# mFinn27/Template-Matching-and-Regression-MapReduce

Hardware: AMD Instinct MI355X
Metric: images/sec (whole node) match+regress+NMS; % HBM/MFMA roofline at 1/2/4/8 GPU (higher is better)
Workload: dtype fp32; 1 GPU; config B: 64x SAM feats 256x64x64 (->128x128), 3 exemplars, templates 3x3-15x15, fp32, cls 0.1, IoU 0.5; config=B, images_per_gpu=64, exemplars=3, parallelism=dp1, decoder=split, decoder_precision=fp32

## Files before the change

### template-matching-and-regression-mapreduce_amd/csrc/conv_split.hip

```cpp
#include <algorithm>
#include <type_traits>

#include "tmr_common.h"

namespace {

typedef _Float16 h8 __attribute__((ext_vector_type(8)));
typedef __bf16 b8 __attribute__((ext_vector_type(8)));
typedef float f32x4 __attribute__((ext_vector_type(4)));
typedef __bf16 b4 __attribute__((ext_vector_type(4)));
typedef __attribute__((address_space(3))) void *lds_ptr_t;


constexpr int BM = 128;
constexpr int TH = 16;
constexpr int TW = 32;
constexpr int LDS_KB = 160;
constexpr int PXG = 8, NG = 4;
constexpr int NWAVES = 8;
constexpr int NTHREADS = NWAVES * 64;
constexpr int WNS = (NWAVES == 8 || TH == 8) ? 2 : 1;
static_assert(TH == 4 * NWAVES / WNS, "a wave owns 4 output rows");
constexpr int NIN = 8 / WNS;
constexpr int ACCW = NIN * 8 * 64 * 4;
// ... 537 lines not shown
#pragma unroll
            for (int q = 0; q < 4; ++q)
                head_fma(head_act((f2){acc[in][2 * q][r], acc[in][2 * q + 1][r]}, inv2, bn2, a.leaky), hw2, hs2[q]);
            __builtin_amdgcn_sched_barrier(0);
        }
    float X[40];
#pragma unroll
    for (int q = 0; q < 4; ++q)
#pragma unroll
        for (int k = 0; k < NHEAD; ++k) {
            X[2 * (5 * q + k)] = hs2[q][k].x;
            X[2 * (5 * q + k) + 1] = hs2[q][k].y;
        }
    float Y[20], Z[10];
#pragma unroll
    for (int m = 0; m < 20; ++m) {
        const auto s = __builtin_amdgcn_permlane16_swap(__float_as_uint(X[2 * m]), __float_as_uint(X[2 * m + 1]),
                                                         false, false);
        Y[m] = __uint_as_float(s[0]) + __uint_as_float(s[1]);
    }
#pragma unroll
    for (int p = 0; p < 10; ++p) {
        const auto s = __builtin_amdgcn_permlane32_swap(__float_as_uint(Y[2 * p]), __float_as_uint(Y[2 * p + 1]),
                                                         false, false);
        Z[p] = __uint_as_float(s[0]) + __uint_as_float(s[1]);
    }
    __syncthreads();
    if (WNS == 2 && wn == 1) {
#pragma unroll
        for (int p = 0; p < 10; ++p) red[((wpix * 10 + p) * 4 + kg) * 16 + l16] = Z[p];
    }
    __syncthreads();
    if (wn == 0) {
#pragma unroll
        for (int p = 0; p < 10; ++p) {
            const int j = 4 * p + kg, m = j >> 1, q = m / NHEAD, k = m - q * NHEAD;
            const int jp = 2 * q + (j & 1);
            const int y = ty0 + wpix * 4 + (jp >> 1), x = tx0 + (jp & 1) * 16 + l16;
            const float v = Z[p] + (WNS == 2 ? red[((wpix * 10 + p) * 4 + kg) * 16 + l16] : 0.0f);
            if (y < a.H && x < a.W) a.partials[(((size_t)nt * NHEAD + k) * a.U + u) * HW + (size_t)y * a.W + x] = v;
        }
    }
}

template <int KS, int PREC, int EPI>
int launch_split(SArgs a, hipStream_t s) {
    constexpr size_t lds = Geo<KS, PREC>::LDS;
    static_assert(lds <= 160 * 1024, "LDS");
    static_assert((4 * 8 * NHEAD * 16 + BM * (NHEAD + 1)) * 4 <= lds, "epilogue scratch");
    auto kern = split_conv_kernel<KS, PREC, EPI>;
    if (tmr_set_max_lds((const void *)kern, lds) !=
        hipSuccess)
        return TMR_E_HIP;
    const int64_t blocks = (int64_t)a.NTW * a.MT * a.U;
    if (blocks <= 0) return TMR_OK;
    TMR_REQUIRE(blocks < (1ll << 31));
    hipLaunchKernelGGL(kern, dim3((unsigned)blocks), dim3(NTHREADS), lds, s, a);
    TMR_CHECK_LAUNCH();
    return TMR_OK;
}

template <int KS, int EPI>
int dispatch_prec(int prec, const SArgs &a, hipStream_t s) {
    switch (prec) {
        case TMR_PREC_F16X3: return launch_split<KS, TMR_PREC_F16X3, EPI>(a, s);
        case TMR_PREC_BF16: return launch_split<KS, TMR_PREC_BF16, EPI>(a, s);
        case TMR_PREC_F16: return launch_split<KS, TMR_PREC_F16, EPI>(a, s);
        default: return TMR_E_INVALID;
    }
}

template <int EPI>
int dispatch_ks(int ks, int prec, const SArgs &a, hipStream_t s) {
    switch (ks) {
        case 1: return dispatch_prec<1, EPI>(prec, a, s);
        case 3: return dispatch_prec<3, EPI>(prec, a, s);
        case 5: return dispatch_prec<5, EPI>(prec, a, s);
        case 7: return dispatch_prec<7, EPI>(prec, a, s);
        default: return TMR_E_INVALID;
    }
}

constexpr int PT = TMR_POINTS_TILE;
constexpr int PCG = PT / 16;
static_assert(PT == 64 && 4 * PT <= NTHREADS, "points tile: one gather lane per point");

struct PArgs {
    SArgs s;
    const float *head_bias;
    const float *box;
    const int32_t *tiles;
    float *b;
};

template <int KS, int PREC>
__global__ __launch_bounds__(NTHREADS) void split_points_kernel(PArgs pa) {
    typedef Prec<PREC> PR;
    typedef typename PR::V V;
    constexpr int T = KS * KS, HALVES = PR::HALVES, WREC = PR::WREC;
    constexpr int NF = BM / 16;
    constexpr int NS = HALVES == 2 ? 3 * T : T;
    const SArgs &a = pa.s;
    constexpr int BB = T * P * PT * 16;
    extern __shared__ __attribute__((aligned(16))) char plds[];
    char *Bs = plds;
    float(*red)[4][PT] = reinterpret_cast<float(*)[4][PT]>(plds + 2 * BB);

    const int tid = threadIdx.x;
    const int lane = tid & 63;
    const int wave = __builtin_amdgcn_readfirstlane(tid >> 6);
    const int l16 = lane & 15, kg = lane >> 4;
    const int HW = a.H * a.W;
    const int32_t *tl = pa.tiles + 3 * (size_t)blockIdx.x;
    const int u = min(max(tl[0], 0), a.U - 1);
    const int first = min(max(tl[1], 0), HW - 1), cnt = min(max(tl[2], 0), PT);
    const int img = a.unit_image ? a.unit_image[u] : u;
    const int NC = a.NC0 + a.NC1;
    const bool active = wave < a.NTW;
    const int nt = a.NT0 + (active ? wave : 0);
    const int *pixi = reinterpret_cast<const int *>(pa.box) + 4 * (size_t)u * HW;
    auto pixel = [&](int p) { return min(max(pixi[4 * (size_t)min(first + (p < cnt ? p : 0), HW - 1)], 0), HW - 1); };

    {
        int py[PCG], px[PCG];
#pragma unroll
        for (int j = 0; j < PCG; ++j) {
            const int pix = pixel(j * 16 + l16);
            py[j] = pix / a.W;
            px[j] = pix - py[j] * a.W;
        }
        const uint32_t cstride = (uint32_t)a.Hp * a.Wp * XREC;
        const int h0 = a.NC0 * HALVES, h1 = a.NC1 * HALVES;
        const __amdgpu_buffer_rsrc_t xr0 = __builtin_amdgcn_make_buffer_rsrc(
            (void *)(h0 ? a.x0 + (size_t)img * h0 * cstride : a.x1), (short)0, h0 * cstride, 0x00020000);
        const __amdgpu_buffer_rsrc_t xr1 = __builtin_amdgcn_make_buffer_rsrc(
            (void *)(h1 ? a.x1 + (size_t)u * h1 * cstride : a.x0), (short)0, h1 * cstride, 0x00020000);
        const uint32_t tapstride = (uint32_t)NC * a.Npad * WREC;
        const __amdgpu_buffer_rsrc_t wr = __builtin_amdgcn_make_buffer_rsrc(
            (void *)a.wp, (short)0, T * tapstride, 0x00020000);
        const uint32_t aoff = (uint32_t)kg * a.Npad * 16 + ((uint32_t)nt * BM + l16) * 16;
        uint32_t goff;
        {
            const int pix = pixel(lane), y = pix / a.W;
            goff = (uint32_t)(y * a.Wp + (pix - y * a.W)) * 16;
        }
        const uint32_t qstride = (uint32_t)a.Hp * a.Wp * 16;
        auto gather = [&](int hc) {
            const bool s0 = hc < h0;
            const uint32_t hs_ = (uint32_t)(s0 ? hc : hc - h0) * cstride;
#pragma unroll
            for (int m = 0; m < (T * P + NWAVES - 1) / NWAVES; ++m) {
                const int i = wave + NWAVES * m;
                if (i < T * P) {
                    const int tap = i / P, q = i % P, ky = tap / KS, kx = tap % KS;
                    buffer_lds16(s0 ? xr0 : xr1, (lds_ptr_t)(Bs + (hc & 1) * BB + i * (PT * 16)), goff,
                                 hs_ + q * qstride + (uint32_t)(ky * a.Wp + kx) * 16);
                }
            }
        };
        const int bfo = kg * (PT * 16) + l16 * 16;
        auto bfrag = [&](int hc, int tap, int j) -> V {
            return *reinterpret_cast<const V *>(Bs + (hc & 1) * BB + tap * (P * PT * 16) + bfo + j * 256);
        };
        gather(0);

        const float sxw = split_sxw<PREC>(a, u);
        f32x4 acc[NF][PCG];
        if (a.acc_init) {
            const int islab = (a.flags & TMR_SPLIT_INIT_BCAST) ? 0 : img;
            const bool i16 = a.flags & TMR_SPLIT_INIT_BF16;
#pragma unroll
            for (int j = 0; j < PCG; ++j) {
                const int mt = (py[j] / TH) * a.TXN + px[j] / TW;
                const int wpix = (py[j] % TH) >> 2, jp = ((py[j] & 3) << 1) | ((px[j] % TW) >> 4);
                const size_t g4 = (((((size_t)islab * a.NT + nt) * a.MT + mt) * NWAVES + wpix * WNS) * ACCW) / 4 +
                                  jp * 64 + kg * 16 + (px[j] & 15);
                if (i16) {
                    const b4 *ai = reinterpret_cast<const b4 *>(a.acc_init) + g4;
#pragma unroll
                    for (int f = 0; f < NF; ++f)
                        acc[f][j] = __builtin_convertvector(ai[(f / NIN) * (ACCW / 4) + (f % NIN) * 8 * 64], f32x4) * sxw;
                } else {
                    const f32x4 *ai = reinterpret_cast<const f32x4 *>(a.acc_init) + g4;
#pragma unroll
                    for (int f = 0; f < NF; ++f)
                        acc[f][j] = ai[(f / NIN) * (ACCW / 4) + (f % NIN) * 8 * 64] * sxw;
                }
            }
        } else {
#pragma unroll
            for (int f = 0; f < NF; ++f)
#pragma unroll
                for (int j = 0; j < PCG; ++j) acc[f][j] = (f32x4){0.0f, 0.0f, 0.0f, 0.0f};
        }

        auto st_part = [](int s) { return HALVES == 2 && s >= 2 * T ? 1 : 0; };
        auto st_tap = [](int s) { return HALVES == 2 ? (s >= 2 * T ? s - 2 * T : s / 2) : s; };
        auto st_term = [](int s) { return HALVES == 2 && s < 2 * T ? s & 1 : 0; };
        auto st_newb = [](int s) { return !(HALVES == 2 && s < 2 * T && (s & 1)); };
        auto st_first = [](int s) { return s == 0 || (HALVES == 2 && s == 2 * T); };
        auto st_last = [](int s) { return s == NS - 1 || (HALVES == 2 && s == 2 * T - 1); };
        V an[NF], bn[PCG];
        auto load_stage = [&](int c, int s) {
            const int tap = st_tap(s);
            const uint32_t as = (uint32_t)tap * tapstride + (uint32_t)c * a.Npad * WREC +
                                (uint32_t)st_term(s) * 4 * a.Npad * 16;
#pragma unroll
            for (int f = 0; f < NF; ++f) an[f] = buffer_load16<V>(wr, aoff + f * 256, as);
            if (st_newb(s) && !st_first(s)) {
#pragma unroll
                for (int j = 0; j < PCG; ++j) bn[j] = bfrag(c * HALVES + st_part(s), tap, j);
            }
        };
        load_stage(0, 0);
        asm volatile("s_waitcnt vmcnt(0)" ::: "memory");
        __syncthreads();
        V bc[PCG];
        const int NHC = NC * HALVES;
        for (int c = 0; c < NC; ++c) {
#pragma unroll
            for (int s = 0; s < NS; ++s) {
                const int hc = c * HALVES + st_part(s);
                V ac[NF];
#pragma unroll
                for (int f = 0; f < NF; ++f) ac[f] = an[f];
                if (st_first(s)) {
                    if (hc + 1 < NHC) gather(hc + 1);
#pragma unroll
                    for (int j = 0; j < PCG; ++j) bc[j] = bfrag(hc, st_tap(s), j);
                } else if (st_newb(s)) {
#pragma unroll
                    for (int j = 0; j < PCG; ++j) bc[j] = bn[j];
                }
                if (s + 1 < NS)
                    load_stage(c, s + 1);
                else
                    load_stage(c + 1 < NC ? c + 1 : c, 0);
                __builtin_amdgcn_sched_barrier(0);
#pragma unroll
                for (int j = 0; j < PCG; ++j)
#pragma unroll
                    for (int f = 0; f < NF; ++f) acc[f][j] = mma(ac[f], bc[j], acc[f][j]);
                __builtin_amdgcn_sched_barrier(0);
                if (st_last(s)) {
                    asm volatile("s_waitcnt vmcnt(0)" ::: "memory");
                    __syncthreads();
                }
            }
        }

        const float inv = 1.0f / sxw;
        const f2 inv2 = {inv, inv};
        f2 hs[WNS][PCG / 2][NHEAD];
#pragma unroll
        for (int w = 0; w < WNS; ++w)
#pragma unroll
            for (int q = 0; q < PCG / 2; ++q)
#pragma unroll
                for (int k = 0; k < NHEAD; ++k) hs[w][q][k] = (f2){0.0f, 0.0f};
#pragma unroll
        for (int f = 0; f < NF; ++f)
#pragma unroll
            for (int r = 0; r < 4; ++r) {
                const int n = nt * BM + f * 16 + 4 * kg + r;
                const float bv = n < a.N ? a.bias[n] : 0.0f;
                const f2 bn2 = {bv, bv};
                f2 hw2[NHEAD];
#pragma unroll
                for (int k = 0; k < NHEAD; ++k) {
                    const float h = a.headw[(size_t)n * NHEAD + k];
                    hw2[k] = (f2){h, h};
                }
#pragma unroll
                for (int q = 0; q < PCG / 2; ++q)
                    head_fma(head_act((f2){acc[f][2 * q][r], acc[f][2 * q + 1][r]}, inv2, bn2, a.leaky), hw2,
                             hs[f / NIN][q]);
            }
#pragma unroll
        for (int q = 0; q < PCG / 2; ++q)
#pragma unroll
            for (int k = 0; k < 4; ++k)
#pragma unroll
                for (int e = 0; e < 2; ++e) {
                    float z[WNS];
#pragma unroll
                    for (int w = 0; w < WNS; ++w) {
                        const float x = hs[w][q][k][e];
                        const float y = x + __shfl_xor(x, 16);
                        z[w] = y + __shfl_xor(y, 32);
                    }
                    if (kg == 0 && active) red[wave][k][(2 * q + e) * 16 + l16] = WNS == 2 ? z[0] + z[1] : z[0];
                }
    }
    __syncthreads();
    if (tid < 4 * PT) {
        const int k = tid / PT, p = tid % PT;
        if (p < cnt) {
            const int pix = pixel(p);
            float s = 0.0f;
            for (int t = 0; t < a.NTW; ++t) s += red[t][k][p];
            pa.b[((size_t)u * 4 + k) * HW + pix] = s + pa.head_bias[k];
        }
    }
}

template <int PREC>
int launch_points(const PArgs &pa, int ntiles, hipStream_t s) {
    constexpr size_t lds = 2 * 9 * P * PT * 16 + NWAVES * 4 * PT * sizeof(float);
    auto kern = split_points_kernel<3, PREC>;
    if (tmr_set_max_lds((const void *)kern, lds) != hipSuccess) return TMR_E_HIP;
    hipLaunchKernelGGL(kern, dim3((unsigned)ntiles), dim3(NTHREADS), lds, s, pa);
    TMR_CHECK_LAUNCH();
    return TMR_OK;
}

inline int prec_halves(int prec) { return prec == TMR_PREC_F16X3 ? 2 : 1; }
inline int prec_wrec(int prec) { return prec == TMR_PREC_F16X3 ? 128 : 64; }
inline bool prec_ok(int prec) {
    return prec == TMR_PREC_F16X3 || prec == TMR_PREC_BF16 || prec == TMR_PREC_F16;
}
inline bool ks_ok(int ks) { return ks == 1 || ks == 3 || ks == 5 || ks == 7; }
inline bool tile_window(int flags, int NT, int &first, int &count) {
    first = (flags >> TMR_SPLIT_TILE_FIRST_SHIFT) & 0xff;
    count = (flags >> TMR_SPLIT_TILE_COUNT_SHIFT) & 0x7f;
    if (count == 0) {
        if (first != 0) return false;
        count = NT;
    }
    return first + count <= NT;
}
inline int pad_h(int H, int ks) { return (int)tmr_cdiv(H, TH) * TH + ks - 1; }
inline int pad_w(int W, int ks) { return (int)tmr_cdiv(W, TW) * TW + ks - 1; }

__device__ __forceinline__ void absmax_commit(float m, unsigned *out) {
    __shared__ float red[4];
    for (int o = 32; o > 0; o >>= 1) m = fmaxf(m, __shfl_xor(m, o));
    if ((threadIdx.x & 63) == 0) red[threadIdx.x >> 6] = m;
    __syncthreads();
    if (threadIdx.x == 0) atomicMax(out, __float_as_uint(fmaxf(fmaxf(red[0], red[1]), fmaxf(red[2], red[3]))));
}

__global__ __launch_bounds__(256) void absmax_rows_kernel(const float *__restrict__ x, int64_t n, int vec,
                                                          unsigned *__restrict__ out) {
    const float *xr = x + (size_t)blockIdx.y * n;
    float m = 0.0f;
    const int64_t step = (int64_t)gridDim.x * blockDim.x;
    if (vec) {
        const float4 *x4 = reinterpret_cast<const float4 *>(xr);
        for (int64_t i = (int64_t)blockIdx.x * blockDim.x + threadIdx.x; i < n / 4; i += step) {
            const float4 v = x4[i];
            m = fmaxf(m, fmaxf(fmaxf(fabsf(v.x), fabsf(v.y)), fmaxf(fabsf(v.z), fabsf(v.w))));
        }
    } else {
        for (int64_t i = (int64_t)blockIdx.x * blockDim.x + threadIdx.x; i < n; i += step)
            m = fmaxf(m, fabsf(xr[i]));
    }
    absmax_commit(m, out + blockIdx.y);
}

constexpr int PA_PIX = 64, PA_GRP = 8;
__global__ __launch_bounds__(PA_PIX * PA_GRP) void pixel_absmax_kernel(const float *__restrict__ x, int S, int C,
                                                                       int64_t HW, float *__restrict__ out) {
    __shared__ float part[PA_GRP][PA_PIX];
    const int lane = threadIdx.x & (PA_PIX - 1), grp = threadIdx.x / PA_PIX;
    const int64_t i = (int64_t)blockIdx.x * PA_PIX + lane;
    float m = 0.0f;
    if (i < (int64_t)S * HW) {
        const int64_t s = i / HW, p = i - s * HW;
        const float *xp = x + (size_t)s * C * HW + p;
#pragma unroll 8
        for (int c = grp; c < C; c += PA_GRP) m = fmaxf(m, fabsf(xp[(size_t)c * HW]));
    }
    part[grp][lane] = m;
    __syncthreads();
    if (grp == 0 && i < (int64_t)S * HW) {
#pragma unroll
        for (int g = 1; g < PA_GRP; ++g) m = fmaxf(m, part[g][lane]);
        out[i] = m;
    }
}

__global__ __launch_bounds__(256) void scale_merge_kernel(const float *__restrict__ img_max,
                                                          const float *__restrict__ unit_max,
                                                          const int32_t *__restrict__ unit_image, int U,
                                                          float *__restrict__ out_img,
                                                          float *__restrict__ out_unit) {
    __shared__ float red[4];
    const int b = blockIdx.x;
    float m = 0.0f;
    for (int u = threadIdx.x; u < U; u += blockDim.x)
        if (unit_image[u] == b) m = fmaxf(m, unit_max[u]);
    for (int o = 32; o > 0; o >>= 1) m = fmaxf(m, __shfl_xor(m, o));
    if ((threadIdx.x & 63) == 0) red[threadIdx.x >> 6] = m;
    __syncthreads();
// ... 371 lines not shown
}

extern "C" int tmr_split_wpack(const float *w, int N, int C0, int C1, int ks, int prec,
                               const float *wmax, void *out, void *stream) {
    TMR_REQUIRE(w && out && N > 0 && C0 >= 0 && C1 >= 0 && C0 + C1 > 0 && ks_ok(ks) && prec_ok(prec));
    TMR_REQUIRE(prec == TMR_PREC_BF16 || wmax);
    const int NC0 = (int)tmr_cdiv(C0, CCH), NC = NC0 + (int)tmr_cdiv(C1, CCH);
    const int Npad = (int)tmr_cdiv(N, BM) * BM;
    const int64_t total = (int64_t)ks * ks * NC * Npad;
    const dim3 grid((unsigned)tmr_cdiv(total, 256)), blk(256);
    hipStream_t s = tmr_stream(stream);
    switch (prec) {
        case TMR_PREC_F16X3:
            hipLaunchKernelGGL(wpack_kernel<TMR_PREC_F16X3>, grid, blk, 0, s, w, N, C0, C1, ks, NC0,
                               NC, Npad, wmax, static_cast<h8 *>(out));
            break;
        case TMR_PREC_BF16:
            hipLaunchKernelGGL(wpack_kernel<TMR_PREC_BF16>, grid, blk, 0, s, w, N, C0, C1, ks, NC0,
                               NC, Npad, nullptr, static_cast<b8 *>(out));
            break;
        default:
            hipLaunchKernelGGL(wpack_kernel<TMR_PREC_F16>, grid, blk, 0, s, w, N, C0, C1, ks, NC0,
                               NC, Npad, wmax, static_cast<h8 *>(out));
            break;
    }
    TMR_CHECK_LAUNCH();
    return TMR_OK;
}

extern "C" int tmr_split_conv(const void *xp0, int C0, const int32_t *unit_image, const void *xp1, int C1, int U,
                              int H, int W, int ks, int prec, const void *wpack, const float *wmax, const float *xmax,
                              const float *bias, int N, int leaky, const float *headw, const float *acc_init,
                              float *out, int flags, void *stream) {
    TMR_REQUIRE(out);
    if (!headw)
        return split_common(xp0, C0, unit_image, xp1, C1, U, H, W, ks, prec, wpack, wmax, xmax, bias, N, leaky,
                            acc_init, out, nullptr, nullptr, 0, flags, stream);
    TMR_REQUIRE(!(flags & TMR_SPLIT_TILED_OUT));
    return split_common(xp0, C0, unit_image, xp1, C1, U, H, W, ks, prec, wpack, wmax, xmax, bias, N, leaky, acc_init,
                        nullptr, headw, out, 1, flags, stream);
}

extern "C" int tmr_split_conv_points(const void *xp0, int C0, const int32_t *unit_image, const void *xp1, int C1,
                                     int U, int H, int W, int ks, int prec, const void *wpack, const float *wmax,
                                     const float *xmax, const float *bias, int N, int leaky, const float *headw,
                                     const float *head_bias, const float *acc_init, const float *box,
                                     const int32_t *tiles, int ntiles, float *b, int flags, void *stream) {
    TMR_REQUIRE(prec_ok(prec) && ks_ok(ks));
    TMR_REQUIRE(wpack && bias && headw && head_bias && box && b && U > 0 && H > 0 && W > 0 && N > 0);
    TMR_REQUIRE(C0 >= 0 && C1 >= 0 && C0 + C1 > 0 && (C0 == 0 || xp0) && (C1 == 0 || xp1));
    TMR_REQUIRE(prec == TMR_PREC_BF16 || (wmax && xmax));
    TMR_REQUIRE(ntiles >= 0 && (ntiles == 0 || tiles));
    TMR_REQUIRE(!(flags & (TMR_SPLIT_TILED_OUT | TMR_SPLIT_OUT_BF16 | TMR_SPLIT_XMAX_PER_PIXEL)));
    TMR_REQUIRE(!acc_init || (flags & TMR_SPLIT_TILED_INIT));
    TMR_REQUIRE(!(flags & TMR_SPLIT_INIT_BF16) || ((flags & TMR_SPLIT_TILED_INIT) && prec != TMR_PREC_F16X3));
    TMR_REQUIRE((int64_t)H * W < (1ll << 29));
    PArgs pa = {};
    SArgs &a = pa.s;
    a.x0 = static_cast<const char *>(xp0);
    a.x1 = static_cast<const char *>(xp1);
    a.unit_image = unit_image;
    a.wp = static_cast<const char *>(wpack);
    a.wmax = prec == TMR_PREC_BF16 ? nullptr : wmax;
    a.xmax = prec == TMR_PREC_BF16 ? nullptr : xmax;
    a.bias = bias;
    a.headw = headw;
    a.acc_init = acc_init;
    a.NC0 = (int)tmr_cdiv(C0, CCH);
    a.NC1 = (int)tmr_cdiv(C1, CCH);
    a.U = U;
    a.H = H;
    a.W = W;
    a.N = N;
    a.NT = (int)tmr_cdiv(N, BM);
    a.Npad = a.NT * BM;
    a.TXN = (int)tmr_cdiv(W, TW);
    a.MT = a.TXN * (int)tmr_cdiv(H, TH);
    a.Hp = pad_h(H, ks);
    a.Wp = pad_w(W, ks);
    a.leaky = leaky;
    a.flags = flags & 0xff;
    a.EI = 1;
    TMR_REQUIRE(tile_window(flags, a.NT, a.NT0, a.NTW));
    if (ks != 3 || a.NTW > NWAVES) return TMR_E_UNSUPPORTED;
    pa.head_bias = head_bias;
    pa.box = box;
    pa.tiles = tiles;
    pa.b = b;
    if (ntiles == 0) return TMR_OK;
    hipStream_t s = tmr_stream(stream);
    switch (prec) {
        case TMR_PREC_F16X3: return launch_points<TMR_PREC_F16X3>(pa, ntiles, s);
        case TMR_PREC_BF16: return launch_points<TMR_PREC_BF16>(pa, ntiles, s);
        default: return launch_points<TMR_PREC_F16>(pa, ntiles, s);
    }
}
```

### template-matching-and-regression-mapreduce_amd/engine.py

```python
from __future__ import annotations

import contextlib
import weakref
from dataclasses import dataclass
from typing import Dict, Optional, Sequence, Tuple

import numpy as np
import torch

from . import exp_table, graphs, host
from ._lib import (PEAKS_DECODE_ONLY, PEAKS_FIND_ONLY, PEAKS_PROB_SCRATCH, POINTS_TILE, PREC_CODES, SPLIT_OUT_BF16,
                   SPLIT_TILED_OUT, SPLIT_XMAX_PER_PIXEL, UNIT_DTYPE, XCORR_ALGOS, TMRError, call, ptr, require_gpu,
                   size, stream, xcorr)
from .decoder_plan import SCALES_FTM, SCALES_MERGED, HeadsLaunch, decoder_plan
from .graphs import _clone_outputs, _GraphBook, _h2d, _units_to_device
from .operands import absmax
from .operands import (absmax_rows, conv2d_split, fold_proj, pack_split_up, pack_split_w, pack_split_x, pixel_absmax,
                       prec_code, scale_merge)
from .xcorr_cost import mfma_fits, xcorr_choice

NHEAD = 5
NMS_SMALL = 256


# ... 266 lines not shown
        self.last_xcorr_flops = float(np.sum(2.0 * C * (H - ht + 1) * (W - wt + 1) * ht * wt))
        self.last_xcorr_bytes = 2.0 * 4 * C * H * W * U
        nimg = len(set(int(i) for i in unit_image))
        self.last_xcorr_dram_bytes = float(C * H * W) * (4.0 * nimg + (2.0 if out16 else 4.0) * U)
        self._memo_absmax(out, "ftm", lambda: slots)
        return out, relu

    def decode(self, fp: torch.Tensor, f_tm: torch.Tensor, unit_image: Sequence[int],
               feats: Optional[torch.Tensor] = None, box_later: bool = False):
        cfg = self.cfg
        ui = _h2d(np.asarray(unit_image, np.int32), f_tm.device, tag="unit_image")
        if cfg.decoder_num_layer != 1:
            return self._decode_stack(fp, f_tm, ui)
        U, C1, H, W = f_tm.shape
        B, dev = fp.shape[0], f_tm.device
        ks, prec, pc = cfg.decoder_kernel_size, cfg.precision, prec_code(cfg.precision)
        p = decoder_plan(cfg, self.fold_proj, self.share_fp_half, self.reuse_image_work, feats is not None, U, B,
                         unit_image, box_later, self._box_tiles() if box_later else 0)
        Cfp = fp.shape[1] if cfg.fusion else 0
        wp, bias, N, Cw, hw, hb, split, wbias = self._fused_decoders(Cfp if p.share else 0, p.fold)
        if Cw != Cfp + C1:
            raise TMRError(f"decoders expect {Cw} input channels, got {Cfp + C1}")
        C0 = feats.shape[1] if p.fold else Cfp
        bplane = self._bias_plane(wbias, H, W) if p.fold else None
        xmax1 = None if p.unscaled else self._memo_absmax(f_tm, "ftm", lambda: absmax_rows(f_tm))
        xp0 = xmax0 = acc0 = None
        if p.scales != SCALES_FTM:
            xmax0 = None if p.unscaled else self._feat_absmax(feats) if p.fold else absmax_rows(fp)
            if p.scales == SCALES_MERGED and not p.unscaled:
                xmax0, xmax1 = scale_merge(xmax0, xmax1, ui, B)
            if p.share and p.fold:
                acc0 = self._acc0_lookup(feats, split, H, W)
            if acc0 is None:
                xp0 = pack_split_up(feats, cfg.feature_upsample, ks, prec, xmax0, ones=False) if p.fold else \
                    pack_split_x(fp, ks, prec, xmax0)
        xp1 = pack_split_x(f_tm, ks, prec, xmax1)
        if p.share:
            wp_fp, wp, zero_b = split
            if acc0 is None:
                acc0 = torch.empty(size("acc", B, N, H, W), device=dev, dtype=torch.float32)
                call("tmr_split_conv", ptr(xp0), C0, None, None, 0, B, H, W, ks, pc, ptr(wp_fp[0]), ptr(wp_fp[1]),
                     ptr(xmax0), ptr(zero_b), N, 0, None, ptr(bplane), ptr(acc0), p.fp_flags, stream())
                if p.fold and self.reuse_image_work:
                    self._acc0_store(feats, split, H, W, acc0)
        part = torch.empty(size("heads_partials", N, U, H, W), device=dev, dtype=torch.float32)
        heads = HeadsLaunch(xp0=None if p.share else xp0, C0=0 if p.share else C0, ui=ui, xp1=xp1, C1=C1, U=U, H=H, W=W,
                            ks=ks, pc=pc, wp=wp, xmax1=xmax1, bias=bias, N=N, hw=hw, hb=hb,
                            a0=acc0 if p.share else bplane, part=part, plan=p)
        first, count = p.window((N + 127) // 128)
        with _timed(self.decoder_events):
            heads.run(first, count)
        n_run = 128 * count if box_later else N
        self.last_decoder_flops = 2.0 * H * W * n_run * (heads.C0 + C1) * ks ** 2 * U
        self.last_shared_flops = 2.0 * H * W * N * C0 * ks ** 2 * B if p.share else 0.0
        self.last_decoder_algo = "split"
        ob = torch.empty(U * (5 if cfg.box_reg else 1) * H * W, device=dev, dtype=torch.float32)
        o = ob[:U * H * W].view(U, 1, H, W)
        b = ob[U * H * W:].view(U, 4, H, W) if cfg.box_reg else None
        call("tmr_heads_reduce", ptr(part[first * NHEAD * U * H * W:]), n_run, 128, U, H, W, ptr(hb), ptr(o),
             None if box_later else ptr(b), stream())
        if box_later:
            heads.b = b
            self._box_ctx = heads
        return o, b

    def _decode_stack(self, fp, f_tm, ui):
        cfg = self.cfg
        x0 = torch.cat([fp.index_select(0, ui.long()), f_tm], 1) if cfg.fusion else f_tm
        res = {}
        for pre in (["decoder_b"] if cfg.box_reg else []) + ["decoder_o"]:
            x = x0
            for l, (w, bb) in enumerate(self._dec_layers(pre)):
                x = self._conv(f"{pre}.{l}", x, w, bb, True)
            res[pre] = x
        ow, ob = self.P["objectness_head.head.0.weight"], self.P["objectness_head.head.0.bias"]
        o = self._conv("obj", res["decoder_o"], ow, ob, False)
        b = None
        if cfg.box_reg:
            lw, lb = self.P["ltrbs_head.head.0.weight"], self.P["ltrbs_head.head.0.bias"]
            b = self._conv("ltrbs", res["decoder_b"], lw, lb, False)
        return o, b

    box_at_peaks = "auto"
    BOX_POINTS_CROSSOVER = {"fp32": 0.40, "bf16": 0.28, "f16": 0.28}

    def _box_tiles(self) -> int:
        return int(self.P["decoder_b.layer.0.weight"].shape[0]) // 128

    def box_at_peaks_ok(self) -> bool:
        cfg = self.cfg
        if self.box_at_peaks == "never" or cfg.decoder_num_layer != 1 or not cfg.box_reg or \
                cfg.decoder_kernel_size != 3 or self.reuse_image_work:
            return False
        if self.box_at_peaks not in ("auto", "always"):
            raise TMRError("box_at_peaks must be 'auto', 'always' or 'never'")
        nb = int(self.P["decoder_b.layer.0.weight"].shape[0])
        return nb % 128 == 0 and 1 <= nb // 128 <= 8

    def box_at_points(self, box: torch.Tensor, tiles: np.ndarray) -> None:
        if len(tiles):
            td = _h2d(np.ascontiguousarray(tiles, np.int32).reshape(-1), box.device)
            self._box_ctx.run_points(box, td, len(tiles))

    def box_dense(self) -> None:
        h = self._box_ctx
        nbt = h.plan.skip_tiles
        h.run(0, nbt)
        scratch_o = torch.empty(h.U * h.H * h.W, device=h.b.device, dtype=torch.float32)
        call("tmr_heads_reduce", ptr(h.part), 128 * nbt, 128, h.U, h.H, h.W, ptr(h.hb), ptr(scratch_o), ptr(h.b),
             stream())

    def _detect_box_at_peaks(self, feats, unit_image, boxes, params):
        r = self._forward_units_eager(feats, [int(i) for i in unit_image], boxes, box_later=True)
        o, b = r["o"], r["b"]
        U, _, H, W = o.shape
        logits, box, ref, counts, _ = self.peaks(o, None, params, want_prob=False, phase="find")
        counts_host = counts.cpu().numpy()
        need = np.where(params["mode"] != 2, counts_host, 0)
        self.last_points = int(need.sum())
        dense = self.box_at_peaks == "auto" and \
            self.last_points > self.BOX_POINTS_CROSSOVER[self.cfg.precision] * U * H * W
        self.last_box_route = "dense" if dense else "points"
        if dense:
            self.box_dense()
            self.last_points_flops = 0.0
        else:
            tiles = host.point_tiles(need, POINTS_TILE)
            self.box_at_points(box, tiles)
            h = self._box_ctx
            self.last_points_flops = 2.0 * 128 * h.plan.skip_tiles * (h.C0 + h.C1) * h.ks ** 2 * POINTS_TILE * len(tiles)
        self._box_ctx = None
        self.peaks(o, b, params, want_prob=False, phase="decode", found=(logits, box, ref, counts))
        return logits, box, ref, counts, counts_host

    def _proj_key(self):
        params = (self.P["input_proj.0.weight"], self.P["input_proj.0.bias"])
        return params, (_version_key(params), self.cfg.precision, self.cfg.feature_upsample)

    def _bind_memo(self, feats: torch.Tensor, fp, split=None, size_=None, acc0=None):
        params, pkey = self._proj_key()
        self._memo = _ImageMemo(weakref.ref(feats), feats._version, feats.data_ptr(), pkey,
                                tuple(weakref.ref(t) for t in params), fp, split, size_, acc0)

    def _fp_lookup(self, feats: torch.Tensor):
        m = self._memo
        params, pkey = self._proj_key()
        hit = m is not None and m.is_for(feats) and m.fp is not None and m.pkey == pkey and \
            all(r() is t for r, t in zip(m.params, params))
        return m.fp if hit else None

    def _acc0_lookup(self, feats, split, H, W):
        m = self._memo
        hit = self.reuse_image_work and m is not None and m.is_for(feats) and m.split is split and m.size == (H, W)
        return m.acc0 if hit else None

    def _acc0_store(self, feats, split, H, W, acc0):
        m = self._memo
        if m is not None and m.is_for(feats):
            m.split, m.size, m.acc0 = split, (H, W), acc0
        else:
            self._bind_memo(feats, None, split, (H, W), acc0)

    def _memo_hit(self, feats: torch.Tensor) -> Optional[_ImageMemo]:
        return self._memo if self._fp_lookup(feats) is not None and self._memo.acc0 is not None else None

    def _forward_units_graphed(self, feats, unit_image, unit_boxes, want_aux):
        if not (self.use_graphs and feats.is_cuda and len(unit_image) <= self.GRAPH_MAX_UNITS) or \
# ... 295 lines not shown
```

Measured before the change: 702.8 images/s.

## Restructure box-at-points kernel: two tiles per block, wave-split channels, weight ring

The points kernel now handles two point tiles per block (128 points). Waves are split by 64-channel half and by tile, with a cross-wave LDS exchange to combine the head partial sums. Gathers load contiguous kx runs per ky row, and a three-deep register ring of weight fragments with counted waits replaces the single lookahead. The aim is to halve weight traffic per point and overlap loads with MFMA. The fp32/bf16/f16 crossover thresholds are raised so the points path is chosen more often, which adds a second pass when more than four N-tiles are active and increases LDS use.

After: 710.1 images/s (median of 6 runs). 1.01x the previous value.

```diff
diff --git a/profiles/points_crossover.py b/profiles/points_crossover.py
--- /dev/null
+++ b/profiles/points_crossover.py
@@ -0,0 +1,76 @@
+import json
+import os
+import sys
+
+import numpy as np
+import torch
+
+REPO = os.path.dirname(os.path.dirname(os.path.abspath(__file__)))
+sys.path.insert(0, REPO)
+import bench
+from tmr_amd import synth
+
+tmr = bench.tmr
+
+
+def events(fn, reps=3):
+    out = []
+    for _ in range(reps):
+        s, e = torch.cuda.Event(enable_timing=True), torch.cuda.Event(enable_timing=True)
+        s.record()
+        fn()
+        e.record()
+        e.synchronize()
+        out.append(s.elapsed_time(e))
+    return out
+
+
+def measure(config):
+    cfg = bench.CONFIGS[config]
+    dev = torch.device("cuda", 0)
+    H = W = 2 * cfg["hf"]
+    prec = cfg.get("precision", "fp32")
+    eng = tmr.TMREngine(synth.reference_state_dict(0, device=dev), tmr.PathConfig(precision=prec))
+    eng.use_graphs = False
+    eng.box_at_peaks = "always"
+    B, E = cfg["batch"], cfg["E"]
+    feats = torch.from_numpy(synth.sam_features(1000, B, bench.CIN, H // 2, W // 2)).to(dev)
+    ex, _ = synth.exemplar_set(2000, B, E, H, W, cfg["kmin"], cfg["kmax"])
+    eng.detect(feats, ex, cls_ths=cfg["cls"], iou_threshold=cfg["iou"])
+    rec = {}
+    points, dense = eng.box_at_points, eng.box_dense
+
+    def both(box, tiles):
+        rec["points_ms_all"] = events(lambda: points(box, tiles))
+        rec["dense_ms_all"] = events(dense)
+        rec["tiles"] = len(tiles)
+        points(box, tiles)
+
+    eng.box_at_points = both
+    eng.detect(feats, ex, cls_ths=cfg["cls"], iou_threshold=cfg["iou"])
+    torch.cuda.synchronize()
+    assert eng.last_box_route == "points" and "tiles" in rec
+    n, pixels = eng.last_points, B * E * H * W
+    pm, dm = min(rec["points_ms_all"]), min(rec["dense_ms_all"])
+    direct = eng.last_points_flops / (pm * 1e-3) / 1e12
+    out = dict(points=n, pixels=pixels, fraction=n / pixels, tiles=rec["tiles"], points_ms=pm, dense_ms=dm,
+               ns_per_point=pm * 1e6 / n, ns_per_pixel=dm * 1e6 / pixels,
+               crossover=(dm / pixels) / (pm / n), points_direct_tflops=direct,
+               points_executed_tflops=direct * bench.SPLIT_TERMS[prec],
+               points_ms_all=rec["points_ms_all"], dense_ms_all=rec["dense_ms_all"])
+    return out
+
+
+def main():
+    out_path = sys.argv[1]
+    res = {}
+    for c in sys.argv[2:] or ["B", "C", "D", "E"]:
+        res[c] = measure(c)
+        print(c, json.dumps({k: res[c][k] for k in ("points", "points_ms", "dense_ms", "crossover")}), flush=True)
+        with open(out_path, "w") as f:
+            json.dump(res, f, indent=1)
+    assert all(np.isfinite(r["crossover"]) for r in res.values())
+
+
+if __name__ == "__main__":
+    main()
diff --git a/template-matching-and-regression-mapreduce_amd/csrc/conv_split.hip b/template-matching-and-regression-mapreduce_amd/csrc/conv_split.hip
--- a/template-matching-and-regression-mapreduce_amd/csrc/conv_split.hip
+++ b/template-matching-and-regression-mapreduce_amd/csrc/conv_split.hip
@@ -643,14 +643,18 @@
 }
 
 constexpr int PT = TMR_POINTS_TILE;
-constexpr int PCG = PT / 16;
-static_assert(PT == 64 && 4 * PT <= NTHREADS, "points tile: one gather lane per point");
+constexpr int PP = 2 * PT;
+constexpr int PCG = PP / 16;
+constexpr int PTW = NWAVES / WNS;
+static_assert(PT == 64 && 4 * PP == NTHREADS, "points block: one store lane per head and point");
+static_assert(WNS == 2 && NWAVES == 2 * P, "points block: a wave per 64-channel half; gathers dealt by (piece, half)");
 
 struct PArgs {
     SArgs s;
     const float *head_bias;
     const float *box;
     const int32_t *tiles;
+    int ntiles;
     float *b;
 };
 
@@ -659,93 +663,110 @@
     typedef Prec<PREC> PR;
     typedef typename PR::V V;
     constexpr int T = KS * KS, HALVES = PR::HALVES, WREC = PR::WREC;
-    constexpr int NF = BM / 16;
+    constexpr int NF = NIN;
     constexpr int NS = HALVES == 2 ? 3 * T : T;
     const SArgs &a = pa.s;
-    constexpr int BB = T * P * PT * 16;
+    constexpr int BB = T * P * PP * 16;
     extern __shared__ __attribute__((aligned(16))) char plds[];
     char *Bs = plds;
-    float(*red)[4][PT] = reinterpret_cast<float(*)[4][PT]>(plds + 2 * BB);
+    float(*red)[4][PP] = reinterpret_cast<float(*)[4][PP]>(plds + 2 * BB);
+    float(*xch)[4][PP] = reinterpret_cast<float(*)[4][PP]>(plds + BB);
+    static_assert(PTW * 4 * PP * sizeof(float) <= BB, "the odd waves' sums fit a B buffer");
 
     const int tid = threadIdx.x;
     const int lane = tid & 63;
     const int wave = __builtin_amdgcn_readfirstlane(tid >> 6);
+    const int wh = wave & 1, wt = wave >> 1;
     const int l16 = lane & 15, kg = lane >> 4;
     const int HW = a.H * a.W;
-    const int32_t *tl = pa.tiles + 3 * (size_t)blockIdx.x;
-    const int u = min(max(tl[0], 0), a.U - 1);
-    const int first = min(max(tl[1], 0), HW - 1), cnt = min(max(tl[2], 0), PT);
-    const int img = a.unit_image ? a.unit_image[u] : u;
+    int tu[2], tfirst[2], tcnt[2], timg[2];
+    float sxw[2];
+#pragma unroll
+    for (int hh = 0; hh < 2; ++hh) {
+        const int64_t ti = 2 * (int64_t)blockIdx.x + hh;
+        const bool have = ti < pa.ntiles;
+        const int32_t *tl = pa.tiles + 3 * (have ? ti : ti - hh);
+        tu[hh] = min(max(tl[0], 0), a.U - 1);
+        tfirst[hh] = min(max(tl[1], 0), HW - 1);
+        tcnt[hh] = have ? min(max(tl[2], 0), PT) : 0;
+        timg[hh] = a.unit_image ? a.unit_image[tu[hh]] : tu[hh];
+        sxw[hh] = split_sxw<PREC>(a, tu[hh]);
+    }
     const int NC = a.NC0 + a.NC1;
-    const bool active = wave < a.NTW;
-    const int nt = a.NT0 + (active ? wave : 0);
-    const int *pixi = reinterpret_cast<const int *>(pa.box) + 4 * (size_t)u * HW;
-    auto pixel = [&](int p) { return min(max(pixi[4 * (size_t)min(first + (p < cnt ? p : 0), HW - 1)], 0), HW - 1); };
-
-    {
-        int py[PCG], px[PCG];
-#pragma unroll
-        for (int j = 0; j < PCG; ++j) {
-            const int pix = pixel(j * 16 + l16);
-            py[j] = pix / a.W;
-            px[j] = pix - py[j] * a.W;
-        }
-        const uint32_t cstride = (uint32_t)a.Hp * a.Wp * XREC;
-        const int h0 = a.NC0 * HALVES, h1 = a.NC1 * HALVES;
-        const __amdgpu_buffer_rsrc_t xr0 = __builtin_amdgcn_make_buffer_rsrc(
-            (void *)(h0 ? a.x0 + (size_t)img * h0 * cstride : a.x1), (short)0, h0 * cstride, 0x00020000);
-        const __amdgpu_buffer_rsrc_t xr1 = __builtin_amdgcn_make_buffer_rsrc(
-            (void *)(h1 ? a.x1 + (size_t)u * h1 * cstride : a.x0), (short)0, h1 * cstride, 0x00020000);
-        const uint32_t tapstride = (uint32_t)NC * a.Npad * WREC;
-        const __amdgpu_buffer_rsrc_t wr = __builtin_amdgcn_make_buffer_rsrc(
-            (void *)a.wp, (short)0, T * tapstride, 0x00020000);
-        const uint32_t aoff = (uint32_t)kg * a.Npad * 16 + ((uint32_t)nt * BM + l16) * 16;
-        uint32_t goff;
-        {
-            const int pix = pixel(lane), y = pix / a.W;
-            goff = (uint32_t)(y * a.Wp + (pix - y * a.W)) * 16;
-        }
-        const uint32_t qstride = (uint32_t)a.Hp * a.Wp * 16;
-        auto gather = [&](int hc) {
-            const bool s0 = hc < h0;
-            const uint32_t hs_ = (uint32_t)(s0 ? hc : hc - h0) * cstride;
-#pragma unroll
-            for (int m = 0; m < (T * P + NWAVES - 1) / NWAVES; ++m) {
-                const int i = wave + NWAVES * m;
-                if (i < T * P) {
-                    const int tap = i / P, q = i % P, ky = tap / KS, kx = tap % KS;
-                    buffer_lds16(s0 ? xr0 : xr1, (lds_ptr_t)(Bs + (hc & 1) * BB + i * (PT * 16)), goff,
-                                 hs_ + q * qstride + (uint32_t)(ky * a.Wp + kx) * 16);
-                }
-            }
-        };
-        const int bfo = kg * (PT * 16) + l16 * 16;
-        auto bfrag = [&](int hc, int tap, int j) -> V {
-            return *reinterpret_cast<const V *>(Bs + (hc & 1) * BB + tap * (P * PT * 16) + bfo + j * 256);
-        };
+    auto pixel = [&](int u, int first, int cnt, int p) {
+        const int *pixi = reinterpret_cast<const int *>(pa.box) + 4 * (size_t)u * HW;
+        return min(max(pixi[4 * (size_t)min(first + (p < cnt ? p : 0), HW - 1)], 0), HW - 1);
+    };
+    const int gu = wh ? tu[1] : tu[0], gfirst = wh ? tfirst[1] : tfirst[0], gcnt = wh ? tcnt[1] : tcnt[0];
+    const int gimg = wh ? timg[1] : timg[0];
+
+    const uint32_t cstride = (uint32_t)a.Hp * a.Wp * XREC;
+    const int h0 = a.NC0 * HALVES, h1 = a.NC1 * HALVES;
+    const __amdgpu_buffer_rsrc_t xr0 = __builtin_amdgcn_make_buffer_rsrc(
+        (void *)(h0 ? a.x0 + (size_t)gimg * h0 * cstride : a.x1), (short)0, h0 * cstride, 0x00020000);
+    const __amdgpu_buffer_rsrc_t xr1 = __builtin_amdgcn_make_buffer_rsrc(
+        (void *)(h1 ? a.x1 + (size_t)gu * h1 * cstride : a.x0), (short)0, h1 * cstride, 0x00020000);
+    const uint32_t tapstride = (uint32_t)NC * a.Npad * WREC;
+    const __amdgpu_buffer_rsrc_t wr = __builtin_amdgcn_make_buffer_rsrc(
+        (void *)a.wp, (short)0, T * tapstride, 0x00020000);
+    uint32_t goff[KS];
+#pragma unroll
+    for (int i = 0; i < KS; ++i) {
+        const int g = 64 * i + lane;
+        const int pix = pixel(gu, gfirst, gcnt, g / KS), y = pix / a.W;
+        goff[i] = (uint32_t)(y * a.Wp + (pix - y * a.W) + g % KS) * 16;
+    }
+    const uint32_t qstride = (uint32_t)a.Hp * a.Wp * 16;
+    auto gather = [&](int hc) {
+        const bool s0 = hc < h0;
+        const uint32_t hs_ = (uint32_t)(s0 ? hc : hc - h0) * cstride + wt * qstride;
+#pragma unroll
+        for (int ky = 0; ky < KS; ++ky)
+#pragma unroll
+            for (int i = 0; i < KS; ++i)
+                buffer_lds16(s0 ? xr0 : xr1,
+                             (lds_ptr_t)(Bs + (hc & 1) * BB + (((ky * P + wt) * PP + wh * PT) * KS + 64 * i) * 16), goff[i],
+                             hs_ + (uint32_t)(ky * a.Wp) * 16);
+    };
+    const int bfo = kg * (PP * KS * 16) + l16 * (KS * 16);
+    auto bfrag = [&](int hc, int tap, int j) -> V {
+        return *reinterpret_cast<const V *>(Bs + (hc & 1) * BB + (tap / KS) * (P * PP * KS * 16) + bfo +
+                                            j * (16 * KS * 16) + (tap % KS) * 16);
+    };
+
+    const int npass = a.NTW > PTW ? 2 : 1;
+    for (int pass = 0; pass < npass; ++pass) {
+        const int wtile = pass * PTW + wt;
+        const bool active = wtile < a.NTW;
+        const int nt = a.NT0 + (active ? wtile : 0);
+        const uint32_t aoff = (uint32_t)kg * a.Npad * 16 + ((uint32_t)nt * BM + wh * (BM / 2) + l16) * 16;
         gather(0);
 
-        const float sxw = split_sxw<PREC>(a, u);
         f32x4 acc[NF][PCG];
         if (a.acc_init) {
-            const int islab = (a.flags & TMR_SPLIT_INIT_BCAST) ? 0 : img;
             const bool i16 = a.flags & TMR_SPLIT_INIT_BF16;
 #pragma unroll
             for (int j = 0; j < PCG; ++j) {
-                const int mt = (py[j] / TH) * a.TXN + px[j] / TW;
-                const int wpix = (py[j] % TH) >> 2, jp = ((py[j] & 3) << 1) | ((px[j] % TW) >> 4);
-                const size_t g4 = (((((size_t)islab * a.NT + nt) * a.MT + mt) * NWAVES + wpix * WNS) * ACCW) / 4 +
-                                  jp * 64 + kg * 16 + (px[j] & 15);
+                constexpr int HJ = PCG / 2;
+                const int hh = j / HJ;
+                const int pix = pixel(tu[hh], tfirst[hh], tcnt[hh], (j % HJ) * 16 + l16);
+                const int py = pix / a.W, px = pix - py * a.W;
+                const float sx = sxw[hh];
+                const int islab = (a.flags & TMR_SPLIT_INIT_BCAST) ? 0 : timg[hh];
+                const int mt = (py / TH) * a.TXN + px / TW;
+                const int wpix = (py % TH) >> 2, jp = ((py & 3) << 1) | ((px % TW) >> 4);
+                const size_t g4 = (((((size_t)islab * a.NT + nt) * a.MT + mt) * NWAVES + wpix * WNS + wh) * ACCW) / 4 +
+                                  jp * 64 + kg * 16 + (px & 15);
                 if (i16) {
                     const b4 *ai = reinterpret_cast<const b4 *>(a.acc_init) + g4;
 #pragma unroll
                     for (int f = 0; f < NF; ++f)
-                        acc[f][j] = __builtin_convertvector(ai[(f / NIN) * (ACCW / 4) + (f % NIN) * 8 * 64], f32x4) * sxw;
+                        acc[f][j] = __builtin_convertvector(ai[f * 8 * 64], f32x4) * sx;
                 } else {
                     const f32x4 *ai = reinterpret_cast<const f32x4 *>(a.acc_init) + g4;
 #pragma unroll
                     for (int f = 0; f < NF; ++f)
-                        acc[f][j] = ai[(f / NIN) * (ACCW / 4) + (f % NIN) * 8 * 64] * sxw;
+                        acc[f][j] = ai[f * 8 * 64] * sx;
                 }
             }
         } else {
@@ -761,19 +782,21 @@
         auto st_newb = [](int s) { return !(HALVES == 2 && s < 2 * T && (s & 1)); };
         auto st_first = [](int s) { return s == 0 || (HALVES == 2 && s == 2 * T); };
         auto st_last = [](int s) { return s == NS - 1 || (HALVES == 2 && s == 2 * T - 1); };
-        V an[NF], bn[PCG];
+        constexpr int AR = 3;
+        static_assert(NS % AR == 0 && NS >= AR, "weight ring");
+        V ar[AR][NF];
         auto load_stage = [&](int c, int s) {
-            const int tap = st_tap(s);
-            const uint32_t as = (uint32_t)tap * tapstride + (uint32_t)c * a.Npad * WREC +
+            if (s >= NS) {
+                s -= NS;
+                c = c + 1 < NC ? c + 1 : c;
+            }
+            const uint32_t as = (uint32_t)st_tap(s) * tapstride + (uint32_t)c * a.Npad * WREC +
                                 (uint32_t)st_term(s) * 4 * a.Npad * 16;
 #pragma unroll
-            for (int f = 0; f < NF; ++f) an[f] = buffer_load16<V>(wr, aoff + f * 256, as);
-            if (st_newb(s) && !st_first(s)) {
-#pragma unroll
-                for (int j = 0; j < PCG; ++j) bn[j] = bfrag(c * HALVES + st_part(s), tap, j);
-            }
+            for (int f = 0; f < NF; ++f) ar[s % AR][f] = buffer_load16<V>(wr, aoff + f * 256, as);
         };
-        load_stage(0, 0);
+#pragma unroll
+        for (int s = 0; s < AR - 1; ++s) load_stage(0, s);
         asm volatile("s_waitcnt vmcnt(0)" ::: "memory");
         __syncthreads();
         V bc[PCG];
@@ -782,48 +805,42 @@
 #pragma unroll
             for (int s = 0; s < NS; ++s) {
                 const int hc = c * HALVES + st_part(s);
-                V ac[NF];
-#pragma unroll
-                for (int f = 0; f < NF; ++f) ac[f] = an[f];
+                load_stage(c, s + AR - 1);
                 if (st_first(s)) {
                     if (hc + 1 < NHC) gather(hc + 1);
 #pragma unroll
                     for (int j = 0; j < PCG; ++j) bc[j] = bfrag(hc, st_tap(s), j);
-                } else if (st_newb(s)) {
-#pragma unroll
-                    for (int j = 0; j < PCG; ++j) bc[j] = bn[j];
                 }
-                if (s + 1 < NS)
-                    load_stage(c, s + 1);
-                else
-                    load_stage(c + 1 < NC ? c + 1 : c, 0);
+                const bool nextb = s + 1 < NS && st_newb(s + 1) && !st_first(s + 1);
                 __builtin_amdgcn_sched_barrier(0);
 #pragma unroll
-                for (int j = 0; j < PCG; ++j)
-#pragma unroll
-                    for (int f = 0; f < NF; ++f) acc[f][j] = mma(ac[f], bc[j], acc[f][j]);
+                for (int j = 0; j < PCG; ++j) {
+#pragma unroll
+                    for (int f = 0; f < NF; ++f) acc[f][j] = mma(ar[s % AR][f], bc[j], acc[f][j]);
+                    if (nextb) {
+                        bc[j] = bfrag(hc, st_tap(s + 1), j);
+                        __builtin_amdgcn_sched_barrier(0);
+                    }
+                }
                 __builtin_amdgcn_sched_barrier(0);
                 if (st_last(s)) {
-                    asm volatile("s_waitcnt vmcnt(0)" ::: "memory");
+                    static_assert((AR - 1) * NF == 8 && T > AR - 1, "the counted wait below");
+                    asm volatile("s_waitcnt vmcnt(8)" ::: "memory");
                     __syncthreads();
                 }
             }
         }
 
-        const float inv = 1.0f / sxw;
-        const f2 inv2 = {inv, inv};
-        f2 hs[WNS][PCG / 2][NHEAD];
-#pragma unroll
-        for (int w = 0; w < WNS; ++w)
-#pragma unroll
-            for (int q = 0; q < PCG / 2; ++q)
-#pragma unroll
-                for (int k = 0; k < NHEAD; ++k) hs[w][q][k] = (f2){0.0f, 0.0f};
+        f2 hs[PCG / 2][NHEAD];
+#pragma unroll
+        for (int q = 0; q < PCG / 2; ++q)
+#pragma unroll
+            for (int k = 0; k < NHEAD; ++k) hs[q][k] = (f2){0.0f, 0.0f};
 #pragma unroll
         for (int f = 0; f < NF; ++f)
 #pragma unroll
             for (int r = 0; r < 4; ++r) {
-                const int n = nt * BM + f * 16 + 4 * kg + r;
+                const int n = nt * BM + wh * (BM / 2) + f * 16 + 4 * kg + r;
                 const float bv = n < a.N ? a.bias[n] : 0.0f;
                 const f2 bn2 = {bv, bv};
                 f2 hw2[NHEAD];
@@ -833,44 +850,63 @@
                     hw2[k] = (f2){h, h};
                 }
 #pragma unroll
-                for (int q = 0; q < PCG / 2; ++q)
-                    head_fma(head_act((f2){acc[f][2 * q][r], acc[f][2 * q + 1][r]}, inv2, bn2, a.leaky), hw2,
-                             hs[f / NIN][q]);
+                for (int q = 0; q < PCG / 2; ++q) {
+                    const float inv = 1.0f / sxw[q / (PCG / 4)];
+                    head_fma(head_act((f2){acc[f][2 * q][r], acc[f][2 * q + 1][r]}, (f2){inv, inv}, bn2, a.leaky), hw2,
+                             hs[q]);
+                }
             }
+        float z[PCG / 2][4][2];
 #pragma unroll
         for (int q = 0; q < PCG / 2; ++q)
 #pragma unroll
             for (int k = 0; k < 4; ++k)
 #pragma unroll
                 for (int e = 0; e < 2; ++e) {
-                    float z[WNS];
-#pragma unroll
-                    for (int w = 0; w < WNS; ++w) {
-                        const float x = hs[w][q][k][e];
-                        const float y = x + __shfl_xor(x, 16);
-                        z[w] = y + __shfl_xor(y, 32);
+                    const float x = hs[q][k][e];
+                    const float y = x + __shfl_xor(x, 16);
+                    z[q][k][e] = y + __shfl_xor(y, 32);
+                }
+        if (wh == 1 && kg == 0 && active) {
+#pragma unroll
+            for (int q = 0; q < PCG / 2; ++q)
+#pragma unroll
+                for (int k = 0; k < 4; ++k)
+#pragma unroll
+                    for (int e = 0; e < 2; ++e) xch[wt][k][(2 * q + e) * 16 + l16] = z[q][k][e];
+        }
+        __syncthreads();
+        if (wh == 0 && kg == 0 && active) {
+#pragma unroll
+            for (int q = 0; q < PCG / 2; ++q)
+#pragma unroll
+                for (int k = 0; k < 4; ++k)
+#pragma unroll
+                    for (int e = 0; e < 2; ++e) {
+                        const int p = (2 * q + e) * 16 + l16;
+                        red[wtile][k][p] = z[q][k][e] + xch[wt][k][p];
                     }
-                    if (kg == 0 && active) red[wave][k][(2 * q + e) * 16 + l16] = WNS == 2 ? z[0] + z[1] : z[0];
-                }
+        }
     }
     __syncthreads();
-    if (tid < 4 * PT) {
-        const int k = tid / PT, p = tid % PT;
-        if (p < cnt) {
-            const int pix = pixel(p);
+    {
+        const int k = tid / PP, p = tid % PP, pl = p % PT;
+        if (pl < gcnt) {
+            const int pix = pixel(gu, gfirst, gcnt, pl);
             float s = 0.0f;
             for (int t = 0; t < a.NTW; ++t) s += red[t][k][p];
-            pa.b[((size_t)u * 4 + k) * HW + pix] = s + pa.head_bias[k];
+            pa.b[((size_t)gu * 4 + k) * HW + pix] = s + pa.head_bias[k];
         }
     }
 }
 
 template <int PREC>
 int launch_points(const PArgs &pa, int ntiles, hipStream_t s) {
-    constexpr size_t lds = 2 * 9 * P * PT * 16 + NWAVES * 4 * PT * sizeof(float);
+    constexpr size_t lds = 2 * 9 * P * PP * 16 + NWAVES * 4 * PP * sizeof(float);
+    static_assert(lds <= LDS_KB * 1024, "LDS");
     auto kern = split_points_kernel<3, PREC>;
     if (tmr_set_max_lds((const void *)kern, lds) != hipSuccess) return TMR_E_HIP;
-    hipLaunchKernelGGL(kern, dim3((unsigned)ntiles), dim3(NTHREADS), lds, s, pa);
+    hipLaunchKernelGGL(kern, dim3((unsigned)((ntiles + 1) / 2)), dim3(NTHREADS), lds, s, pa);
     TMR_CHECK_LAUNCH();
     return TMR_OK;
 }
@@ -1408,10 +1444,11 @@
     a.flags = flags & 0xff;
     a.EI = 1;
     TMR_REQUIRE(tile_window(flags, a.NT, a.NT0, a.NTW));
-    if (ks != 3 || a.NTW > NWAVES) return TMR_E_UNSUPPORTED;
+    if (ks != 3 || a.NTW > 2 * PTW) return TMR_E_UNSUPPORTED;
     pa.head_bias = head_bias;
     pa.box = box;
     pa.tiles = tiles;
+    pa.ntiles = ntiles;
     pa.b = b;
     if (ntiles == 0) return TMR_OK;
     hipStream_t s = tmr_stream(stream);
diff --git a/template-matching-and-regression-mapreduce_amd/engine.py b/template-matching-and-regression-mapreduce_amd/engine.py
--- a/template-matching-and-regression-mapreduce_amd/engine.py
+++ b/template-matching-and-regression-mapreduce_amd/engine.py
@@ -372,7 +372,7 @@
         return o, b
 
     box_at_peaks = "auto"
-    BOX_POINTS_CROSSOVER = {"fp32": 0.40, "bf16": 0.28, "f16": 0.28}
+    BOX_POINTS_CROSSOVER = {"fp32": 0.50, "bf16": 0.47, "f16": 0.47}
 
     def _box_tiles(self) -> int:
         return int(self.P["decoder_b.layer.0.weight"].shape[0]) // 128
```
